# EEGKit/yagi

Hardware: AMD Instinct MI355X
Metric: Msamples/sec, 256-tap firfilt_crcf + 4096-pt FFT stream (higher is better)
Workload: dtype f32

## Files before the change

yagi_amd/csrc/capi.hip:

```cpp
#include <cmath>
#include <cstdlib>
#include <complex>
#include <memory>

#include <algorithm>
#include <atomic>

#include "kernels.hpp"
#include "objstate.hpp"

namespace yagi {

int design_kaiser(size_t n, float fc, float as_, float mu, std::vector<float> &h);
int window_value(int type, size_t i, size_t wlen, float arg, float *out);
int design_notch(size_t m, float f0, float as_, std::vector<float> &h);

static int require_device() {
    static int ok = -1;
    if (ok < 0) {
        int n = 0;
        hipError_t e = hipGetDeviceCount(&n);
        ok = (e == hipSuccess && n > 0) ? 1 : 0;
    }
    if (!ok) return fail(YAGI_ERR_DEVICE, "no HIP device available: libyagi_hip has no CPU fallback");
    return YAGI_OK;
}

template <class V> static V one_of();
template <> float one_of<float>() { return 1.0f; }
template <> cf32 one_of<cf32>() { return cf32{1.0f, 0.0f}; }
static cf32 to_c(float v, cf32 *) { return cf32{v, 0.0f}; }
static float to_c(float v, float *) { return v; }

struct StreamPipe {
    bool on = false;
    static constexpr int kLanes = 2;
    hipStream_t lane[kLanes] = {};
    hipEvent_t in = nullptr, done[kLanes] = {};
    bool busy[kLanes] = {};
    unsigned calls = 0;
    const void *prev_tail = nullptr;
    int init() {
        if (lane[0]) return YAGI_OK;
        for (auto &s : lane) YG_HIP(hipStreamCreateWithFlags(&s, hipStreamNonBlocking));
        YG_HIP(hipEventCreateWithFlags(&in, hipEventDisableTiming));
        for (auto &e : done) YG_HIP(hipEventCreateWithFlags(&e, hipEventDisableTiming));
        return YAGI_OK;
    }
    ~StreamPipe() {
        for (auto &s : lane)
            if (s) { (void)hipStreamSynchronize(s); (void)hipStreamDestroy(s); }
        if (in) (void)hipEventDestroy(in);
        for (auto &e : done) if (e) (void)hipEventDestroy(e);
    }
};

template <class T>
struct DevWindow {
    int len = 0;
    static constexpr int kBufs = 3;
    PingPong<kBufs> ring;
    static constexpr size_t kSlack = 4096;
    std::vector<T> hbuf;
    size_t hend = 0;
    Mirror mirror;
    uint64_t npush = 0;
    StreamPipe pipe;

    int join(hipStream_t st) {
        for (int i = 0; i < StreamPipe::kLanes; ++i) {
            if (pipe.busy[i]) YG_HIP(hipStreamWaitEvent(st, pipe.done[i], 0));
            pipe.busy[i] = false;
        }
        if (pipe.prev_tail) {
            YG_TRY(launch_update_window<T>(dev(), static_cast<const T *>(pipe.prev_tail), (size_t)len, len, next(), st));
            flip();
            pipe.prev_tail = nullptr;
        }
        return YAGI_OK;
    }
    int begin_piped(hipStream_t st, hipStream_t *lane, const T **win) {
        const int i = (int)(pipe.calls % (unsigned)StreamPipe::kLanes);
        YG_HIP(hipEventRecord(pipe.in, st));
        YG_HIP(hipStreamWaitEvent(pipe.lane[i], pipe.in, 0));
        *lane = pipe.lane[i];
        *win = pipe.prev_tail ? static_cast<const T *>(pipe.prev_tail) : dev();
        return YAGI_OK;
    }
    int finish_piped(const T *x, size_t n) {
        const int i = (int)(pipe.calls % (unsigned)StreamPipe::kLanes);
        YG_HIP(hipEventRecord(pipe.done[i], pipe.lane[i]));
        pipe.busy[i] = true;
        ++pipe.calls;
        pipe.prev_tail = x + (n - (size_t)len);
        mirror.dev_written();
        return YAGI_OK;
    }
    bool can_pipe(size_t n) const { return pipe.on && mirror.dev_current() && n >= (size_t)len; }

    int init(int n, hipStream_t st) {
        len = n;
        YG_TRY(ring.alloc((size_t)n * sizeof(T)));
        hbuf.assign((size_t)n + kSlack, T{});
        npush = 0;
        return reset(st);
    }
    int reset(hipStream_t st) {
        YG_TRY(join(st));
        YG_HIP(hipMemsetAsync(ring.cur(), 0, (size_t)len * sizeof(T), st));
        std::fill(hbuf.begin(), hbuf.begin() + len, T{});
        hend = (size_t)len;
        mirror.in_sync();
        return YAGI_OK;
    }
    const T *dev() const { return ring.template cur<T>(); }
    T *next() { return ring.template next<T>(); }
    void flip() { ring.flip(); mirror.dev_written(); }
    int advance(const T *x_dev, size_t n, hipStream_t st) {
        if (n == 0) return YAGI_OK;
        YG_TRY(launch_update_window<T>(dev(), x_dev, n, len, next(), st));
        flip();
        return YAGI_OK;
    }
    const T *host() const { return hbuf.data() + (hend - (size_t)len); }
    void push(T v) {
        if (hend == hbuf.size()) {
            std::memmove(hbuf.data(), hbuf.data() + (hend - (size_t)len + 1), ((size_t)len - 1) * sizeof(T));
            hend = (size_t)len - 1;
        }
        hbuf[hend++] = v;
        ++npush;
        mirror.host_written();
    }
    int ensure_dev(hipStream_t st) {
        YG_TRY(join(st));
        return mirror.need_dev([&] { return upload(ring.cur(), host(), (size_t)len * sizeof(T), st); });
    }
    int ensure_host(hipStream_t st) {
        YG_TRY(join(st));
        return mirror.need_host([&] {
            hend = (size_t)len;
            return download(hbuf.data(), ring.cur(), (size_t)len * sizeof(T), st);
        });
    }
    int clone_from(const DevWindow &o, hipStream_t st) {
        YG_TRY(init(o.len, st));
        YG_HIP(hipMemcpyAsync(ring.cur(), o.ring.cur(), (size_t)len * sizeof(T), hipMemcpyDeviceToDevice, st));
        YG_HIP(hipStreamSynchronize(st));
        npush = o.npush;
        mirror.dev_written();
        return YAGI_OK;
    }
};

template <class T, class C> T host_fir_ring_dot(const T *w, size_t L, size_t head, const C *h, C scale);
template <class T, class C> T host_fir_window_dot(const T *w, size_t L, const C *h, C scale);

template <class K>
struct FirFilt {
    using T = typename K::T;
    using C = typename K::C;
    hipStream_t st = nullptr;
    int L = 0, Lp = 0;
    std::vector<C> h;
    C scale = one_of<C>();
    DevBuf taps;
    DevBuf taps_pad;
    DevBuf apack;
    int Lm = 0;
    DevBuf hfreq, twf, twb;
    DevBuf gfft, gfft_s;
    DevBuf hfreq_s;
    bool hfreq_s_valid = false;
    float hfreq_s_scale = 0.f;
    bool conv_ready = false;
    DevWindow<T> w;
    Staging ws;
    int kernel_choice = 0;
    int prepare_conv();

    int load_taps(const C *hh, size_t n) {
        if (n == 0) return fail(YAGI_ERR_CONFIG, "filter length must be greater than zero");
        if (n > (size_t)1 << 24) return fail(YAGI_ERR_CONFIG, "filter too long");
        h.assign(hh, hh + n);
        L = (int)n;
        YG_TRY(fill(taps, h.data(), n * sizeof(C), st));
        conv_ready = false;
        hfreq_s_valid = false;
        if (K::id == 1) {
            Lp = (L + 31) / 32 * 32;
            std::vector<float> hp((size_t)Lp, 0.0f);
            std::memcpy(hp.data(), h.data(), n * sizeof(float));
            YG_TRY(fill(taps_pad, hp.data(), (size_t)Lp * sizeof(float), st));
            Lm = mfma_lp_for(L);
            if (Lm) {
                std::vector<float> ap(toeplitz_pack_floats(Lm));
                pack_toeplitz_taps(reinterpret_cast<const float *>(h.data()), L, Lm, ap.data());
                YG_TRY(fill(apack, ap.data(), ap.size() * sizeof(float), st));
            }
        }
        return YAGI_OK;
    }
    int init(const C *hh, size_t n) {
        YG_TRY(require_device());
        YG_TRY(load_taps(hh, n));
        return w.init(L, st);
    }
    int block_dev(const T *x, size_t n, T *y);
    T host_execute() const {
        const size_t Ls = (size_t)L, head = (Ls - (size_t)(w.npush % Ls)) % Ls;
        return host_fir_ring_dot<T, C>(w.host(), Ls, head, h.data(), scale);
    }
};

template <class K>
int FirFilt<K>::block_dev(const T *x, size_t n, T *y) {
    if (n == 0) return w.ensure_dev(st);
    const bool piped = w.can_pipe(n) && (kernel_choice != 4 || conv_ready);
    hipStream_t s = st;
    const T *win = nullptr;
    if (piped) YG_TRY(w.begin_piped(st, &s, &win));
    else { YG_TRY(w.ensure_dev(st)); win = w.dev(); }
    T *wnext = piped ? nullptr : w.next();
    w.npush += n;
    const bool conv = kernel_choice == 4 && L <= 2049;
    if (conv) {
        YG_TRY(prepare_conv());
        if constexpr (K::id == 0)
            YG_TRY(launch_fir_rrrf_fftconv(win, x, 0, n, hfreq.as<cf32>(), scale, L, twf.as<cf32>(), twb.as<cf32>(), y, n, s, wnext));
        else
            YG_TRY(launch_fir_cccf_fftconv(win, x, 0, n, hfreq.as<cf32>(), scale, L, twf.as<cf32>(), twb.as<cf32>(), y, n, s, wnext));
    } else {
        YG_TRY((launch_fir_block<K>(win, x, taps.template as<C>(), L, 1, scale, y, n, s, 0, wnext)));
    }
    if (piped) return w.finish_piped(x, n);
    w.flip();
    return YAGI_OK;
}
template <>
int FirFilt<CRCF>::block_dev(const cf32 *x, size_t n, cf32 *y) {
    if (n == 0) return w.ensure_dev(st);
    const bool conv = kernel_choice == 4 && L <= 2049;
    const bool mfma = Lm && (kernel_choice == 3 || (kernel_choice == 0 && n >= ((size_t)1 << 16)));
// ... 1790 lines not shown
        if (q->use_conv) {                                                                          \
            YG_TRY(q->fir.w.ensure_dev(q->st));                                                          \
            YG_TRY(o->fir.w.clone_from(q->fir.w, q->st));                                           \
        } else {                                                                                    \
            YG_HIP(hipMemcpyAsync(o->w.cur(), q->w.cur(), (size_t)q->n * sizeof(cf32),              \
                                  hipMemcpyDeviceToDevice, q->st));                                 \
        YG_HIP(hipStreamSynchronize(q->st));                                                    \
        }                                                                                           \
        *out = o.release();                                                                         \
        return YAGI_OK;                                                                             \
    } catch (...) { return ::yagi::api_exception(); }                                               \
    int yagi_hip_fftfilt_##K##_set_stream(yagi_hip_fftfilt_##K q, yagi_stream_t s) try {            \
        CHECK_Q(q);                                                                                 \
        if (q->st == to_stream(s)) return YAGI_OK;                                                  \
        YG_HIP(hipStreamSynchronize(q->st));                                                        \
        q->st = to_stream(s);                                                                       \
        return YAGI_OK;                                                                             \
    } catch (...) { return ::yagi::api_exception(); }                                               \
    int yagi_hip_fftfilt_##K##_reset(yagi_hip_fftfilt_##K q) try {                                  \
        CHECK_Q(q);                                                                                 \
        return q->reset();                                                                          \
    } catch (...) { return ::yagi::api_exception(); }                                               \
    int yagi_hip_fftfilt_##K##_set_scale(yagi_hip_fftfilt_##K q, C scale) try {                     \
        CHECK_Q(q);                                                                                 \
        q->scale = div_scalar(scale, 2.0f * (float)q->n);                                           \
        return YAGI_OK;                                                                             \
    } catch (...) { return ::yagi::api_exception(); }                                               \
    int yagi_hip_fftfilt_##K##_get_scale(yagi_hip_fftfilt_##K q, C *scale) try {                    \
        CHECK_Q(q);                                                                                 \
        CHECK_PTR(scale);                                                                           \
        *scale = mul_scalar(q->scale, 2.0f * (float)q->n);                                          \
        return YAGI_OK;                                                                             \
    } catch (...) { return ::yagi::api_exception(); }                                               \
    int yagi_hip_fftfilt_##K##_get_length(yagi_hip_fftfilt_##K q, size_t *h_len) try {              \
        CHECK_Q(q);                                                                                 \
        CHECK_PTR(h_len);                                                                           \
        *h_len = q->h.size();                                                                       \
        return YAGI_OK;                                                                             \
    } catch (...) { return ::yagi::api_exception(); }                                               \
    int yagi_hip_fftfilt_##K##_execute(yagi_hip_fftfilt_##K q, const T *x, size_t nx, T *y,         \
                                       size_t ny) try {                                             \
        CHECK_Q(q);                                                                                 \
        if (nx != (size_t)q->n || ny != (size_t)q->n)                                               \
            return fail(YAGI_ERR_CONFIG, "input and output lengths must match filter block size");  \
        CHECK_PTR(x);                                                                               \
        CHECK_PTR(y);                                                                               \
        return q->blocks_host(x, 1, y);                                                             \
    } catch (...) { return ::yagi::api_exception(); }                                               \
    int yagi_hip_fftfilt_##K##_execute_blocks(yagi_hip_fftfilt_##K q, const T *x, size_t nblocks,   \
                                              T *y) try {                                           \
        CHECK_Q(q);                                                                                 \
        if (nblocks == 0) return YAGI_OK;                                                           \
        CHECK_PTR(x);                                                                               \
        CHECK_PTR(y);                                                                               \
        return q->blocks_host(x, nblocks, y);                                                       \
    } catch (...) { return ::yagi::api_exception(); }                                               \
    int yagi_hip_fftfilt_##K##_execute_blocks_dev(yagi_hip_fftfilt_##K q, const T *x,               \
                                                  size_t nblocks, T *y) try {                       \
        CHECK_Q(q);                                                                                 \
        if (nblocks == 0) return YAGI_OK;                                                           \
        CHECK_PTR(x);                                                                               \
        CHECK_PTR(y);                                                                               \
        CHECK_NOALIAS(x, nblocks * (size_t)q->n, y, nblocks * (size_t)q->n);                        \
        return q->blocks_dev(x, nblocks, y);                                                        \
    } catch (...) { return ::yagi::api_exception(); }                                               \
    }

YAGI_FFTFILT_IMPL(rrrf, RRRF, float, float)
YAGI_FFTFILT_IMPL(crcf, CRCF, yagi_cf32, float)
YAGI_FFTFILT_IMPL(cccf, CCCF, yagi_cf32, yagi_cf32)

struct yagi_hip_firfft_crcf_s : FirFft {};

extern "C" {

int yagi_hip_firfft_crcf_create(const float *h, size_t h_len, size_t nfft, yagi_hip_firfft_crcf *q) try {
    CHECK_PTR(q);
    *q = nullptr;
    if (h_len && !h) return fail(YAGI_ERR_CONFIG, "null pointer argument");
    if (nfft == 0) return fail(YAGI_ERR_CONFIG, "fft length must be greater than zero");
    auto o = std::make_unique<yagi_hip_firfft_crcf_s>();
    YG_TRY(o->fir.init(h, h_len));
    if (o->fir.L > 2049) return fail(YAGI_ERR_CONFIG, "fused stream: filter too long (%zu taps, at most 2049)", h_len);
    o->nfft = nfft;
    if (nfft == 4096) YG_TRY(make_stream_twiddles(o->tw));
    else YG_TRY(fft_plan_init(o->plan, nfft, YAGI_FFT_FORWARD));
    *q = o.release();
    return YAGI_OK;
} catch (...) { return ::yagi::api_exception(); }
int yagi_hip_firfft_crcf_destroy(yagi_hip_firfft_crcf q) try { delete q; return YAGI_OK; } catch (...) { return ::yagi::api_exception(); }
int yagi_hip_firfft_crcf_set_pipeline(yagi_hip_firfft_crcf q, int on) try {
    CHECK_Q(q);
    YG_TRY(q->join());
    if (on) YG_TRY(q->fir.w.pipe.init());
    q->fir.w.pipe.on = on != 0;
    return YAGI_OK;
} catch (...) { return ::yagi::api_exception(); }
int yagi_hip_firfft_crcf_join(yagi_hip_firfft_crcf q) try {
    CHECK_Q(q);
    return q->join();
} catch (...) { return ::yagi::api_exception(); }
int yagi_hip_firfft_crcf_set_stream(yagi_hip_firfft_crcf q, yagi_stream_t s) try {
    CHECK_Q(q);
    if (q->fir.st == to_stream(s)) return YAGI_OK;
    YG_TRY(q->join());
    YG_HIP(hipStreamSynchronize(q->fir.st));
    q->fir.st = to_stream(s);
    return YAGI_OK;
} catch (...) { return ::yagi::api_exception(); }
int yagi_hip_firfft_crcf_set_scale(yagi_hip_firfft_crcf q, float scale) try { CHECK_Q(q); q->fir.scale = scale; return YAGI_OK; } catch (...) { return ::yagi::api_exception(); }
int yagi_hip_firfft_crcf_reset(yagi_hip_firfft_crcf q) try {
    CHECK_Q(q);
    YG_TRY(q->join());
    return q->fir.w.reset(q->fir.st);
} catch (...) { return ::yagi::api_exception(); }
int yagi_hip_firfft_crcf_set_variant(yagi_hip_firfft_crcf q, int variant) try {
    CHECK_Q(q);
    if (variant < 0 || variant > 4) return fail(YAGI_ERR_CONFIG, "unknown variant %d", variant);
    if (q->nfft != 4096 && variant != 0 && variant != 3)
        return fail(YAGI_ERR_CONFIG, "nfft = %zu runs as overlap-save FIR + batched FFT (variant 3) only", q->nfft);
    if (variant == 3 && q->fir.L > 2049) return fail(YAGI_ERR_CONFIG, "fast convolution needs <= 2049 taps");
    if (variant == 4 && q->fir.L > 257) return fail(YAGI_ERR_CONFIG, "frequency-domain variant needs <= 257 taps");
    if (variant == 2 && !q->fir.Lm) return fail(YAGI_ERR_CONFIG, "MFMA variant needs <= 256 taps");
    if (variant == 1 && q->fir.Lp > kSlideMaxTaps) return fail(YAGI_ERR_CONFIG, "sliding variant needs <= %d taps", kSlideMaxTaps);
    YG_TRY(q->join());
    q->variant = variant;
    return YAGI_OK;
} catch (...) { return ::yagi::api_exception(); }
int yagi_hip_firfft_crcf_execute_dev(yagi_hip_firfft_crcf q, const yagi_cf32 *x, size_t nframes, yagi_cf32 *spectra) try {
    CHECK_Q(q);
    if (nframes == 0) return YAGI_OK;
    CHECK_PTR(x);
    CHECK_PTR(spectra);
    CHECK_NOALIAS(x, nframes * q->nfft, spectra, nframes * q->nfft);
    auto &f = q->fir;
    const bool use_freq = q->nfft == 4096 && (q->variant == 4 || (q->variant == 0 && f.L <= 257));
    const bool piped = use_freq && f.w.can_pipe(nframes * q->nfft) && f.conv_ready && f.hfreq_s_valid &&
                       f.hfreq_s_scale == f.scale;
    if (!piped) YG_TRY(f.w.ensure_dev(f.st));
    if (q->nfft != 4096) {
        YG_TRY(f.prepare_conv());
        const size_t n = nframes * q->nfft;
        YG_TRY(q->scratch.ensure(n * sizeof(cf32)));
        cf32 *ys = q->scratch.as<cf32>();
        YG_TRY(launch_fir_crcf_fftconv(f.w.dev(), x, 0, n, f.hfreq.as<cf32>(), f.scale, f.L, f.twf.as<cf32>(),
                                       f.twb.as<cf32>(), ys, n, f.st));
        YG_TRY(launch_fft_batch(q->plan.d, ys, spectra, nframes, f.st));
        return f.w.advance(x, n, f.st);
    }
    if (piped) {
        const size_t n = nframes * q->nfft;
        hipStream_t lane;
        const cf32 *win;
        YG_TRY(f.w.begin_piped(f.st, &lane, &win));
        YG_TRY(launch_firfft_crcf_4096_freq(win, x, f.hfreq_s.as<cf32>(), f.gfft_s.as<cf32>(), f.L, q->tw.as<cf32>(), spectra,
                                            nullptr, nframes, lane));
        return f.w.finish_piped(x, n);
    }
    if (use_freq) {
        YG_TRY(f.prepare_conv());
        if (!f.hfreq_s_valid || f.hfreq_s_scale != f.scale) {
            YG_TRY(f.hfreq_s.ensure(4096 * sizeof(cf32)));
            YG_TRY(launch_scale_cf32(f.hfreq.as<cf32>(), f.scale, f.hfreq_s.as<cf32>(), 4096, f.st));
            YG_TRY(f.gfft_s.ensure(512 * sizeof(cf32)));
            YG_TRY(launch_scale_cf32(f.gfft.as<cf32>(), f.scale, f.gfft_s.as<cf32>(), 512, f.st));
            f.hfreq_s_valid = true;
            f.hfreq_s_scale = f.scale;
        }
        YG_TRY(launch_firfft_crcf_4096_freq(f.w.dev(), x, f.hfreq_s.as<cf32>(), f.gfft_s.as<cf32>(), f.L,
                                            q->tw.as<cf32>(), spectra, f.w.next(), nframes, f.st));
        f.w.flip();
        return YAGI_OK;
    }
    const bool use_conv = q->variant == 3 || (q->variant == 0 && f.L <= 2049);
    if (use_conv) {
        YG_TRY(f.prepare_conv());
        const size_t n = nframes * q->nfft;
        YG_TRY(q->scratch.ensure(n * sizeof(cf32)));
        FftPlanDev d;
        d.n = 4096;
        d.dir = YAGI_FFT_FORWARD;
        d.tw = q->tw.as<cf32>();
        cf32 *ys = q->scratch.as<cf32>();
        YG_TRY(launch_fir_crcf_fftconv(f.w.dev(), x, 0, n, f.hfreq.as<cf32>(), f.scale, f.L, f.twf.as<cf32>(),
                                       f.twb.as<cf32>(), ys, n, f.st));
        YG_TRY(launch_fft_batch(d, ys, spectra, nframes, f.st));
        return f.w.advance(x, n, f.st);
    }
    YG_TRY(launch_firfft_crcf_4096(f.w.dev(), x, f.taps_pad.as<float>(), f.apack.as<float>(), f.L, f.Lp, f.Lm, f.scale,
                                   q->tw.as<cf32>(), spectra, nframes, q->variant, f.st));
    return f.w.advance(x, nframes * q->nfft, f.st);
} catch (...) { return ::yagi::api_exception(); }
int yagi_hip_firfft_crcf_execute(yagi_hip_firfft_crcf q, const yagi_cf32 *x, size_t nframes, yagi_cf32 *spectra) try {
    CHECK_Q(q);
    if (nframes == 0) return YAGI_OK;
    CHECK_PTR(x);
    CHECK_PTR(spectra);
    const size_t n = nframes * q->nfft;
    YG_TRY(q->join());
    return q->ws.run(q->fir.st, x, n, spectra, n, [&](const cf32 *xd, cf32 *yd) {
        YG_TRY(yagi_hip_firfft_crcf_execute_dev(q, xd, nframes, yd));
        return q->join();
    });
} catch (...) { return ::yagi::api_exception(); }

}

struct yagi_hip_firpfbch_crcf_s : PfbCh {};
struct yagi_hip_firpfbch2_crcf_s : PfbCh2 {};

extern "C" {

int yagi_hip_firpfbch_crcf_create(size_t M, size_t p, const float *h, yagi_hip_firpfbch_crcf *q) try {
    CHECK_PTR(q);
    *q = nullptr;
    if (M == 0) return fail(YAGI_ERR_CONFIG, "number of channels must be greater than zero");
    if (p == 0) return fail(YAGI_ERR_CONFIG, "invalid filter size (must be greater than 0)");
    CHECK_PTR(h);
    if (M > 8192 || p > 4096) return fail(YAGI_ERR_CONFIG, "channelizer too large");
    YG_TRY(require_device());
    auto o = std::make_unique<yagi_hip_firpfbch_crcf_s>();
    o->M = (int)M;
    o->p = (int)p;
    YG_TRY(fill(o->h, h, M * p * sizeof(float), nullptr));
    YG_TRY(make_twiddles((int)M, YAGI_FFT_FORWARD, o->tw));
    const size_t hl = (p - 1) * M;
    YG_TRY(o->hist.init((int)(hl ? hl : 1), nullptr));
    YG_TRY(o->syn_hist.init((int)(hl ? hl : 1), nullptr));
    *q = o.release();
    return YAGI_OK;
} catch (...) { return ::yagi::api_exception(); }
int yagi_hip_firpfbch_crcf_create_kaiser(size_t M, size_t m, float as_, yagi_hip_firpfbch_crcf *q) try {
    CHECK_PTR(q);
    *q = nullptr;
    if (M == 0) return fail(YAGI_ERR_CONFIG, "number of channels must be greater than zero");
    if (m == 0) return fail(YAGI_ERR_CONFIG, "invalid filter size (must be greater than 0)");
    std::vector<float> hf;
    YG_TRY(design_kaiser(2 * M * m + 1, 0.5f / (float)M, std::fabs(as_), 0.0f, hf));
    return yagi_hip_firpfbch_crcf_create(M, 2 * m, hf.data(), q);
} catch (...) { return ::yagi::api_exception(); }
int yagi_hip_firpfbch_crcf_destroy(yagi_hip_firpfbch_crcf q) try { delete q; return YAGI_OK; } catch (...) { return ::yagi::api_exception(); }
int yagi_hip_firpfbch_crcf_set_stream(yagi_hip_firpfbch_crcf q, yagi_stream_t s) try {
    CHECK_Q(q);
    if (q->st == to_stream(s)) return YAGI_OK;
    YG_HIP(hipStreamSynchronize(q->st));
    q->st = to_stream(s);
    return YAGI_OK;
} catch (...) { return ::yagi::api_exception(); }
int yagi_hip_firpfbch_crcf_reset(yagi_hip_firpfbch_crcf q) try {
    CHECK_Q(q);
    YG_TRY(q->hist.reset(q->st));
    return q->syn_hist.reset(q->st);
} catch (...) { return ::yagi::api_exception(); }
int yagi_hip_firpfbch_crcf_analyzer_execute_dev(yagi_hip_firpfbch_crcf q, const yagi_cf32 *x, size_t nframes, yagi_cf32 *y) try {
    CHECK_Q(q);
    if (nframes == 0) return YAGI_OK;
    CHECK_PTR(x);
    CHECK_PTR(y);
    CHECK_NOALIAS(x, nframes * (size_t)q->M, y, nframes * (size_t)q->M);
    bool written = false;
    cf32 *next = (q->p > 1 && q->hist.len == (int)((q->p - 1) * q->M)) ? q->hist.next() : nullptr;
    YG_TRY(launch_firpfbch(q->hist.dev(), x, q->h.as<float>(), q->M, q->p, q->tw.as<cf32>(), y, nframes, q->st, next, &written));
    if (written) { q->hist.flip(); return YAGI_OK; }
    if (q->p > 1) return q->hist.advance(x, nframes * (size_t)q->M, q->st);
    return YAGI_OK;
} catch (...) { return ::yagi::api_exception(); }
int yagi_hip_firpfbch_crcf_analyzer_execute(yagi_hip_firpfbch_crcf q, const yagi_cf32 *x, size_t nframes, yagi_cf32 *y) try {
    CHECK_Q(q);
    if (nframes == 0) return YAGI_OK;
    CHECK_PTR(x);
    CHECK_PTR(y);
    const size_t n = nframes * (size_t)q->M;
    return q->ws.run(q->st, x, n, y, n,
                     [&](const cf32 *xd, cf32 *yd) { return yagi_hip_firpfbch_crcf_analyzer_execute_dev(q, xd, nframes, yd); });
} catch (...) { return ::yagi::api_exception(); }

int yagi_hip_firpfbch_crcf_synthesizer_execute_dev(yagi_hip_firpfbch_crcf q, const yagi_cf32 *x, size_t nframes, yagi_cf32 *y) try {
    CHECK_Q(q);
    if (nframes == 0) return YAGI_OK;
    CHECK_PTR(x);
    CHECK_PTR(y);
    CHECK_NOALIAS(x, nframes * (size_t)q->M, y, nframes * (size_t)q->M);
    YG_TRY(launch_firpfbch_syn(q->syn_hist.dev(), x, q->h.as<float>(), q->M, q->p, q->tw.as<cf32>(), y, nframes, q->st));
    if (q->p > 1) return q->syn_hist.advance(x, nframes * (size_t)q->M, q->st);
    return YAGI_OK;
} catch (...) { return ::yagi::api_exception(); }
int yagi_hip_firpfbch_crcf_synthesizer_execute(yagi_hip_firpfbch_crcf q, const yagi_cf32 *x, size_t nframes, yagi_cf32 *y) try {
    CHECK_Q(q);
    if (nframes == 0) return YAGI_OK;
    CHECK_PTR(x);
    CHECK_PTR(y);
    const size_t n = nframes * (size_t)q->M;
    return q->ws.run(q->st, x, n, y, n,
                     [&](const cf32 *xd, cf32 *yd) { return yagi_hip_firpfbch_crcf_synthesizer_execute_dev(q, xd, nframes, yd); });
} catch (...) { return ::yagi::api_exception(); }

int yagi_hip_firpfbch2_crcf_create(size_t M, size_t m, const float *h, yagi_hip_firpfbch2_crcf *q) try {
    CHECK_PTR(q);
    *q = nullptr;
    if (M < 2 || (M & 1)) return fail(YAGI_ERR_CONFIG, "number of channels must be greater than 2 and even");
    if (m < 1) return fail(YAGI_ERR_CONFIG, "filter semi-length must be at least 1");
    CHECK_PTR(h);
    if (M > 8192 || m > 2048) return fail(YAGI_ERR_CONFIG, "channelizer too large");
    YG_TRY(require_device());
    auto o = std::make_unique<yagi_hip_firpfbch2_crcf_s>();
    o->M = (int)M;
    o->m = (int)m;
    const size_t hl = 2 * M * m;
    YG_TRY(fill(o->h, h, hl * sizeof(float), nullptr));
    YG_TRY(make_twiddles((int)M, YAGI_FFT_FORWARD, o->tw));
// ... 3653 lines not shown
```

yagi_amd/csrc/devmath.hpp:

```cpp
#pragma once
#include <hip/hip_runtime.h>

#include "common.hpp"

namespace yagi {

template <class T> __device__ __forceinline__ T zero_of();
template <> __device__ __forceinline__ float zero_of<float>() { return 0.0f; }
template <> __device__ __forceinline__ cf32 zero_of<cf32>() { return cf32{0.0f, 0.0f}; }

__device__ __forceinline__ float add(float a, float b) { return a + b; }
__device__ __forceinline__ cf32 add(cf32 a, cf32 b) { return cf32{a.re + b.re, a.im + b.im}; }

__device__ __forceinline__ float mul(float a, float b) { return a * b; }
__device__ __forceinline__ cf32 mul(cf32 a, float b) { return cf32{a.re * b, a.im * b}; }
__device__ __forceinline__ cf32 mul(float a, cf32 b) { return cf32{a * b.re, a * b.im}; }
__device__ __forceinline__ cf32 mul(cf32 a, cf32 b) {
    return cf32{fmaf(a.re, b.re, -a.im * b.im), fmaf(a.re, b.im, a.im * b.re)};
}

__device__ __forceinline__ float mac(float acc, float a, float b) { return fmaf(a, b, acc); }
__device__ __forceinline__ cf32 mac(cf32 acc, cf32 a, float b) {
    return cf32{fmaf(a.re, b, acc.re), fmaf(a.im, b, acc.im)};
}
__device__ __forceinline__ cf32 mac(cf32 acc, float a, cf32 b) {
    return cf32{fmaf(a, b.re, acc.re), fmaf(a, b.im, acc.im)};
}
__device__ __forceinline__ cf32 mac(cf32 acc, cf32 a, cf32 b) {
    return cf32{fmaf(a.re, b.re, fmaf(-a.im, b.im, acc.re)), fmaf(a.re, b.im, fmaf(a.im, b.re, acc.im))};
}

__device__ __forceinline__ float wave_reduce_sum(float v) {
#pragma unroll
    for (int off = 32; off > 0; off >>= 1) v += __shfl_xor(v, off, 64);
    return v;
}
__device__ __forceinline__ cf32 wave_reduce_sum(cf32 v) {
#pragma unroll
    for (int off = 32; off > 0; off >>= 1) {
        v.re += __shfl_xor(v.re, off, 64);
        v.im += __shfl_xor(v.im, off, 64);
    }
    return v;
}

typedef float v2f __attribute__((ext_vector_type(2)));
__device__ __forceinline__ float2 f2(v2f v) { return make_float2(v.x, v.y); }
__device__ __forceinline__ v2f tov(float2 a) { return v2f{a.x, a.y}; }

__device__ __forceinline__ float2 cadd(float2 a, float2 b) { return f2(tov(a) + tov(b)); }
__device__ __forceinline__ float2 csub(float2 a, float2 b) { return f2(tov(a) - tov(b)); }
__device__ __forceinline__ float2 cmul(float2 a, float2 w) {
    v2f r;
    asm("v_pk_mul_f32 %0, %1, %2 op_sel_hi:[0,1]\n\t"
        "v_pk_fma_f32 %0, %1, %2, %0 op_sel:[1,1,0] op_sel_hi:[1,0,1] neg_lo:[0,1,0]"
        : "=&v"(r) : "v"(tov(a)), "v"(tov(w)));
    return f2(r);
}
__device__ __forceinline__ float2 cmul_conj(float2 a, float2 w) {
    v2f r;
    asm("v_pk_mul_f32 %0, %1, %2 op_sel_hi:[0,1] neg_hi:[0,1]\n\t"
        "v_pk_fma_f32 %0, %1, %2, %0 op_sel:[1,1,0] op_sel_hi:[1,0,1]"
        : "=&v"(r) : "v"(tov(a)), "v"(tov(w)));
    return f2(r);
}
template <int SIGN>
__device__ __forceinline__ float2 cmul_dir(float2 a, float2 w) { return SIGN < 0 ? cmul(a, w) : cmul_conj(a, w); }
__device__ __forceinline__ float2 cmul_k(float2 a, float2 k) {
    v2f r;
    asm("v_pk_mul_f32 %0, %1, %2 op_sel_hi:[0,1]\n\t"
        "v_pk_fma_f32 %0, %1, %2, %0 op_sel:[1,1,0] op_sel_hi:[1,0,1] neg_lo:[0,1,0]"
        : "=&v"(r) : "v"(tov(a)), "s"(tov(k)));
    return f2(r);
}
__device__ __forceinline__ float2 cscale(float2 a, float s) { return f2(tov(a) * s); }
__device__ __forceinline__ float2 mul_mi(float2 a) { return make_float2(a.y, -a.x); }
__device__ __forceinline__ float2 mul_pi(float2 a) { return make_float2(-a.y, a.x); }
template <int SIGN>
__device__ __forceinline__ void addsub_rot(float2 a, float2 b, float2 &p, float2 &m) {
    v2f pp, mm;
    if (SIGN < 0) {
        asm("v_pk_add_f32 %0, %1, %2 op_sel:[0,1] op_sel_hi:[1,0] neg_hi:[0,1]" : "=v"(pp) : "v"(tov(a)), "v"(tov(b)));
        asm("v_pk_add_f32 %0, %1, %2 op_sel:[0,1] op_sel_hi:[1,0] neg_lo:[0,1]" : "=v"(mm) : "v"(tov(a)), "v"(tov(b)));
    } else {
        asm("v_pk_add_f32 %0, %1, %2 op_sel:[0,1] op_sel_hi:[1,0] neg_lo:[0,1]" : "=v"(pp) : "v"(tov(a)), "v"(tov(b)));
        asm("v_pk_add_f32 %0, %1, %2 op_sel:[0,1] op_sel_hi:[1,0] neg_hi:[0,1]" : "=v"(mm) : "v"(tov(a)), "v"(tov(b)));
    }
    p = f2(pp);
    m = f2(mm);
}

template <int NT, int B, bool EXACT, class Load, class Store>
__device__ __forceinline__ void batched_for_b(int total, Load load, Store store) {
    using V = decltype(load(0));
    for (int e0 = threadIdx.x; e0 < total; e0 += B * NT) {
        V r[B];
#pragma unroll
        for (int it = 0; it < B; ++it) {
            const int e = e0 + NT * it;
            r[it] = load(EXACT || e < total ? e : total - 1);
        }
#pragma unroll
        for (int it = 0; it < B; ++it) {
            const int e = e0 + NT * it;
            if (EXACT || e < total) store(e, r[it]);
        }
    }
}
template <int NT, class Load, class Store>
__device__ __forceinline__ void batched_for(int total, Load load, Store store) {
    if (total == 8 * NT) batched_for_b<NT, 8, true>(total, load, store);
    else if (total <= 2 * NT) batched_for_b<NT, 2, false>(total, load, store);
    else if (total <= 4 * NT) batched_for_b<NT, 4, false>(total, load, store);
    else batched_for_b<NT, 8, false>(total, load, store);
}

typedef unsigned v2u_t __attribute__((ext_vector_type(2)));
__device__ __forceinline__ __amdgpu_buffer_rsrc_t make_rsrc(const void *p, unsigned bytes) {
    return __builtin_amdgcn_make_buffer_rsrc(const_cast<void *>(p), 0, bytes, 0x00020000);
}
#ifndef YG_STREAM_LD
#define YG_STREAM_LD 16
#endif
#ifndef YG_STREAM_ST
#define YG_STREAM_ST 2
#endif
constexpr int kStreamLoad = YG_STREAM_LD, kStreamStore = YG_STREAM_ST;
__device__ __forceinline__ float2 buf_ld(__amdgpu_buffer_rsrc_t r, unsigned voff, unsigned soff) {
    const v2u_t q = __builtin_amdgcn_raw_buffer_load_b64(r, voff, soff, kStreamLoad);
    return make_float2(__uint_as_float(q.x), __uint_as_float(q.y));
}
template <class T>
__device__ __forceinline__ T ld_stream(const T *p) {
    static_assert(sizeof(T) == 4 || sizeof(T) == 8, "4- or 8-byte samples");
    if constexpr (kStreamLoad == 16) {
        T v;
        if constexpr (sizeof(T) == 4) {
            const unsigned q = __hip_atomic_load(reinterpret_cast<const unsigned *>(p), __ATOMIC_RELAXED, __HIP_MEMORY_SCOPE_AGENT);
            __builtin_memcpy(&v, &q, 4);
        } else {
            const unsigned long long q = __hip_atomic_load(reinterpret_cast<const unsigned long long *>(p), __ATOMIC_RELAXED,
                                                           __HIP_MEMORY_SCOPE_AGENT);
            __builtin_memcpy(&v, &q, 8);
        }
        return v;
    } else {
        return *p;
    }
}
template <class T>
__device__ __forceinline__ void st_stream(T *p, T v) {
    static_assert(sizeof(T) == 4 || sizeof(T) == 8 || sizeof(T) == 16, "4-, 8- or 16-byte samples");
    if constexpr (kStreamStore == 2) {
        typedef float vec_t __attribute__((ext_vector_type(sizeof(T) / 4)));
        vec_t q;
        __builtin_memcpy(&q, &v, sizeof(T));
        __builtin_nontemporal_store(q, reinterpret_cast<vec_t *>(p));
    } else {
        *p = v;
    }
}
template <int AUX>
__device__ __forceinline__ float2 buf_ld_aux(__amdgpu_buffer_rsrc_t r, unsigned voff, unsigned soff) {
    const v2u_t q = __builtin_amdgcn_raw_buffer_load_b64(r, voff, soff, AUX);
    return make_float2(__uint_as_float(q.x), __uint_as_float(q.y));
}
template <int AUX>
__device__ __forceinline__ void buf_st_aux(__amdgpu_buffer_rsrc_t r, unsigned voff, unsigned soff, float2 v) {
    v2u_t q;
    q.x = __float_as_uint(v.x);
    q.y = __float_as_uint(v.y);
    __builtin_amdgcn_raw_buffer_store_b64(q, r, voff, soff, AUX);
}
template <class T>
__device__ __forceinline__ T buf_ld_t(__amdgpu_buffer_rsrc_t r, unsigned voff, unsigned soff) {
    if constexpr (sizeof(T) == 4) {
        const unsigned q = __builtin_amdgcn_raw_buffer_load_b32(r, voff, soff, kStreamLoad);
        T v;
        __builtin_memcpy(&v, &q, 4);
        return v;
    } else {
        static_assert(sizeof(T) == 8, "4- or 8-byte samples");
        const v2u_t q = __builtin_amdgcn_raw_buffer_load_b64(r, voff, soff, kStreamLoad);
        T v;
        __builtin_memcpy(&v, &q, 8);
        return v;
    }
}
__device__ __forceinline__ void buf_st(__amdgpu_buffer_rsrc_t r, unsigned voff, unsigned soff, float2 v) {
    v2u_t q;
    q.x = __float_as_uint(v.x);
    q.y = __float_as_uint(v.y);
    __builtin_amdgcn_raw_buffer_store_b64(q, r, voff, soff, kStreamStore);
}


}
```

yagi_amd/csrc/freq_kernels.hip:

```cpp
#include "fft_core.hpp"
#include "kernels.hpp"

namespace yagi {

constexpr int kFreqMaxTaps = 257;
constexpr unsigned kOffCvs = kFft4096LdsFloat2;
constexpr unsigned kOffT256 = kOffCvs + 256;
constexpr unsigned kFreqLdsFloat2 = kOffT256 + 16 * kTRow;

__device__ __forceinline__ void freq_pass23(float2 (&v)[16], float2 *__restrict__ lds, const float2 *__restrict__ T) {
    const unsigned t = threadIdx.x;
    {
        const unsigned c = t >> 4, bp = t & 15;
#pragma unroll
        for (int a = 0; a < 16; ++a) v[a] = lds[c * kEx1Stride + 16 * a + bp];
        __syncthreads();
        dft16<-1>(v);
#pragma unroll
        for (int cp = 0; cp < 16; ++cp) {
            float2 u = v[dft16_pos(cp)];
            if (cp) u = cmul(u, T[bp * kTRow + cp]);
            lds[bp * kEx2Stride + cp * 16 + c] = u;
        }
    }
    __syncthreads();
    float2 w[16];
#pragma unroll
    for (int bp = 0; bp < 16; ++bp) w[bp] = lds[bp * kEx2Stride + t];
    dft16<-1>(w);
#pragma unroll
    for (int d = 0; d < 16; ++d) v[d] = w[dft16_pos(d)];
    __syncthreads();
}

__device__ __forceinline__ void freq_head256(const float2 *__restrict__ xs, float2 (&v)[16], float2 *__restrict__ lds,
                                             const float2 *__restrict__ T, float2 wbc) {
    const unsigned t = threadIdx.x;
    const unsigned c = t >> 4, bp = t & 15;
    v[0] = xs[bp];
#pragma unroll
    for (int a = 1; a < 16; ++a) v[a] = cmul(xs[16 * a + bp], T[c * kTRow + a]);
    dft16<-1>(v);
#pragma unroll
    for (int cp = 0; cp < 16; ++cp) {
        float2 u = cmul(v[dft16_pos(cp)], wbc);
        if (cp) u = cmul(u, T[bp * kTRow + cp]);
        lds[bp * kEx2Stride + cp * 16 + c] = u;
    }
    __syncthreads();
    float2 w[16];
#pragma unroll
    for (int b = 0; b < 16; ++b) w[b] = lds[b * kEx2Stride + t];
    dft16<-1>(w);
#pragma unroll
    for (int d = 0; d < 16; ++d) v[d] = w[dft16_pos(d)];
}

template <int SIGN>
__device__ __forceinline__ float2 w8(float c, float s) { return make_float2(c, SIGN < 0 ? -s : s); }
template <int SIGN, int NOUT>
__device__ __forceinline__ void dft8_combine(const float2 (&E)[4], float2 (&O)[4], float2 (&X)[8]) {
    const float r2 = 0.70710678118654752f;
    O[1] = cmul_k(O[1], w8<SIGN>(r2, r2));
    O[3] = cmul_k(O[3], w8<SIGN>(-r2, r2));
    X[0] = cadd(E[0], O[0]);
    X[1] = cadd(E[1], O[1]);
    X[3] = cadd(E[3], O[3]);
    if (NOUT > 4) {
        X[4] = csub(E[0], O[0]);
        X[5] = csub(E[1], O[1]);
        X[7] = csub(E[3], O[3]);
        addsub_rot<SIGN>(E[2], O[2], X[2], X[6]);
    } else {
        float2 unused;
        addsub_rot<SIGN>(E[2], O[2], X[2], unused);
    }
}
template <int SIGN, int NIN = 8, int NOUT = 8>
__device__ __forceinline__ void dft8(const float2 (&v)[8], float2 (&X)[8]) {
    float2 E[4], O[4];
    if (NIN == 4) {
        E[0] = cadd(v[0], v[2]); E[2] = csub(v[0], v[2]); addsub_rot<SIGN>(v[0], v[2], E[1], E[3]);
        O[0] = cadd(v[1], v[3]); O[2] = csub(v[1], v[3]); addsub_rot<SIGN>(v[1], v[3], O[1], O[3]);
    } else {
        E[0] = v[0]; E[1] = v[2]; E[2] = v[4]; E[3] = v[6];
        O[0] = v[1]; O[1] = v[3]; O[2] = v[5]; O[3] = v[7];
        dft4<SIGN>(E[0], E[1], E[2], E[3]);
        dft4<SIGN>(O[0], O[1], O[2], O[3]);
    }
    dft8_combine<SIGN, NOUT>(E, O, X);
}
constexpr unsigned kW512S1 = 72, kW512S2 = 68, kW512Ex2 = 8 * kW512S1;
template <int SIGN, int NIN, int NOUT>
__device__ __forceinline__ void wave_fft512(const float2 (&v)[8], float2 (&X)[8], float2 *__restrict__ scr, unsigned l,
                                            float2 w1, float2 w2, float2 w4, float2 u1, float2 u2, float2 u4) {
    float2 z[8], r[8];
    dft8<SIGN, NIN, 8>(v, z);
    {
        const float2 w3 = cmul(w1, w2), w5 = cmul(w4, w1), w6 = cmul(w4, w2), w7 = cmul(w4, w3);
        const float2 w[8] = {w1, w1, w2, w3, w4, w5, w6, w7};
        scr[l] = z[0];
#pragma unroll
        for (int c = 1; c < 8; ++c) scr[c * kW512S1 + l] = cmul_dir<SIGN>(z[c], w[c]);
    }
    __builtin_amdgcn_wave_barrier();
    const unsigned c = l >> 3, bp = l & 7u;
#pragma unroll
    for (int a = 0; a < 8; ++a) r[a] = scr[c * kW512S1 + 8 * a + bp];
    dft8<SIGN, 8, 8>(r, z);
    {
        const float2 u3 = cmul(u1, u2), u5 = cmul(u4, u1), u6 = cmul(u4, u2), u7 = cmul(u4, u3);
        const float2 u[8] = {u1, u1, u2, u3, u4, u5, u6, u7};
        scr[kW512Ex2 + bp * kW512S2 + c] = z[0];
#pragma unroll
        for (int cp = 1; cp < 8; ++cp) scr[kW512Ex2 + bp * kW512S2 + 8 * cp + c] = cmul_dir<SIGN>(z[cp], u[cp]);
    }
    __builtin_amdgcn_wave_barrier();
#pragma unroll
    for (int b = 0; b < 8; ++b) r[b] = scr[kW512Ex2 + b * kW512S2 + l];
    __builtin_amdgcn_wave_barrier();
    dft8<SIGN, 8, NOUT>(r, X);
}

struct CorrOperands {
    float2 dp[4], dq[4];
    float2 w1, w2, w4, u1, u2, u4;
    float2 gc[8];
};
__device__ __forceinline__ void freq_load_corr_fft(CorrOperands &o, const float2 *__restrict__ win,
                                                   const float2 *__restrict__ x, int L, unsigned f,
                                                   const float2 *__restrict__ tw, const float2 *__restrict__ gfft) {
    const unsigned l = threadIdx.x & 63u;
    const int Lc = L - 1;
    const float2 *xf = x + (size_t)f * 4096;
    const float2 *prev = Lc ? (f ? xf - Lc : win + 1) : xf;
    const float2 *own = xf + (4096 - (Lc ? Lc : 1));
#pragma unroll
    for (int a = 0; a < 4; ++a) {
        const unsigned m = 64u * a + l, mi = (int)m < Lc ? m : 0u;
        o.dp[a] = prev[mi];
        o.dq[a] = own[mi];
    }
    o.w1 = tw[8u * l]; o.w2 = tw[16u * l]; o.w4 = tw[32u * l];
    const unsigned bp = l & 7u;
    o.u1 = tw[64u * bp]; o.u2 = tw[128u * bp]; o.u4 = tw[256u * bp];
#pragma unroll
    for (int d = 0; d < 8; ++d) o.gc[d] = gfft[l + 64u * d];
}
__device__ __forceinline__ void freq_correction_fft(const CorrOperands &o, int L, float2 *__restrict__ scr,
                                                    float2 *__restrict__ cvs) {
    const unsigned l = threadIdx.x & 63u;
    const int Lc = L - 1;
    float2 v[8], D[8];
#pragma unroll
    for (int a = 0; a < 4; ++a) v[a] = (int)(64u * a + l) < Lc ? csub(o.dp[a], o.dq[a]) : make_float2(0.f, 0.f);
#pragma unroll
    for (int a = 4; a < 8; ++a) v[a] = make_float2(0.f, 0.f);
    wave_fft512<-1, 4, 8>(v, D, scr, l, o.w1, o.w2, o.w4, o.u1, o.u2, o.u4);
#pragma unroll
    for (int d = 0; d < 8; ++d) v[d] = cmul(D[d], o.gc[d]);
    wave_fft512<1, 8, 4>(v, D, scr, l, o.w1, o.w2, o.w4, o.u1, o.u2, o.u4);
#pragma unroll
    for (int d = 0; d < 4; ++d) cvs[l + 64u * d] = (int)(64u * d + l) < Lc ? D[d] : make_float2(0.f, 0.f);
}

__global__ void __launch_bounds__(256, 4)
firfft_crcf_4096_freq_kernel(const float2 *__restrict__ win, const float2 *__restrict__ x,
                              const float2 *__restrict__ hs, const float2 *__restrict__ gfft, int L,
                              const float2 *__restrict__ tw, float2 *__restrict__ out,
                              float2 *__restrict__ win_next, unsigned nframes) {
    __shared__ __attribute__((aligned(16))) float2 lds[kFreqLdsFloat2];
    float2 *cvs = lds + kOffCvs;
    const float2 *T = lds + kOffT256;
    const float2 *ax = tw + 4096;
    const unsigned t = threadIdx.x, f = blockIdx.x;
    const bool wave0 = __builtin_amdgcn_readfirstlane(t >> 6) == 0;
    const float2 tw_t = ax[1280 + t];
    float2 v[16];
    CorrOperands co;
    if (wave0) freq_load_corr_fft(co, win, x, L, f, tw, gfft);
    __builtin_amdgcn_sched_barrier(0);
    {
        const __amdgpu_buffer_rsrc_t rx = make_rsrc(x + (size_t)f * 4096, 32768u);
#pragma unroll
        for (unsigned a = 0; a < 16; ++a) v[a] = buf_ld(rx, 8u * t, 2048u * a);
    }
    __builtin_amdgcn_sched_barrier(0);
    lds[kOffT256 + (t >> 4) * kTRow + (t & 15u)] = tw_t;
    if (f == nframes - 1 && win_next) {
        const float2 *xf = x + (size_t)f * 4096;
        for (int i = t; i < L; i += 256) win_next[i] = xf[4096 - L + i];
    }
    if (wave0) freq_correction_fft(co, L, lds, cvs);
    __syncthreads();
    dft16<-1>(v);
    {
        float2 w[16];
        twiddle_powers_from(w, ax[t], ax[256 + t], ax[512 + t], ax[768 + t]);
#pragma unroll
        for (int c = 0; c < 16; ++c) {
            float2 z = v[dft16_pos(c)];
            if (c) z = cmul(z, w[c]);
            lds[c * kEx1Stride + t] = z;
        }
    }
    __syncthreads();
    freq_pass23(v, lds, T);
    {
        const __amdgpu_buffer_rsrc_t rh = make_rsrc(hs, 32768u);
        float2 hv[16];
#pragma unroll
        for (unsigned d = 0; d < 16; ++d) hv[d] = buf_ld_aux<0>(rh, 8u * t, 2048u * d);
#pragma unroll
        for (unsigned d = 0; d < 16; ++d) v[d] = cmul(v[d], hv[d]);
    }
    float2 u[16];
    freq_head256(cvs, u, lds, T, ax[1024 + t]);
    const __amdgpu_buffer_rsrc_t ro = make_rsrc(out + (size_t)f * 4096, 32768u);
#pragma unroll
    for (unsigned d = 0; d < 16; ++d)
        buf_st(ro, 8u * t, 2048u * d, make_float2(v[d].x + u[d].x, v[d].y + u[d].y));
}

__global__ void scale_cf32_kernel(const float2 *__restrict__ src, float s, float2 *__restrict__ dst, unsigned n) {
    const unsigned i = blockIdx.x * blockDim.x + threadIdx.x;
    if (i < n) dst[i] = make_float2(src[i].x * s, src[i].y * s);
}
int launch_scale_cf32(const cf32 *src, float s, cf32 *dst, size_t n, hipStream_t st) {
    if (n == 0) return YAGI_OK;
    scale_cf32_kernel<<<(unsigned)((n + 255) / 256), 256, 0, st>>>(reinterpret_cast<const float2 *>(src), s,
                                                                    reinterpret_cast<float2 *>(dst), (unsigned)n);
    YG_LAUNCH_CHECK();
    return YAGI_OK;
}

int launch_firfft_crcf_4096_freq(const cf32 *win, const cf32 *x, const cf32 *hs_scaled, const cf32 *gfft_scaled,
                                 int L, const cf32 *tw_stream, cf32 *spectra, cf32 *win_next, size_t nframes,
                                 hipStream_t st) {
    if (nframes == 0) return YAGI_OK;
    if (L < 1 || L > kFreqMaxTaps)
        return fail(YAGI_ERR_CONFIG, "frequency-domain stream kernel needs 1..%d taps (got %d)", kFreqMaxTaps, L);
    if (nframes > 0x7fffffffull) return fail(YAGI_ERR_CONFIG, "block too large");
    firfft_crcf_4096_freq_kernel<<<(unsigned)nframes, 256, 0, st>>>(
        reinterpret_cast<const float2 *>(win), reinterpret_cast<const float2 *>(x),
        reinterpret_cast<const float2 *>(hs_scaled), reinterpret_cast<const float2 *>(gfft_scaled), L,
        reinterpret_cast<const float2 *>(tw_stream), reinterpret_cast<float2 *>(spectra),
        reinterpret_cast<float2 *>(win_next), (unsigned)nframes);
    YG_LAUNCH_CHECK();
    return YAGI_OK;
}

}
```

Baseline: 303,600.

## Fuse window-tail writes into piped kernel and restructure freq kernel head/tail

```diff
diff --git a/yagi_amd/csrc/capi.hip b/yagi_amd/csrc/capi.hip
--- a/yagi_amd/csrc/capi.hip
+++ b/yagi_amd/csrc/capi.hip
@@ -40,6 +40,7 @@
     bool busy[kLanes] = {};
     unsigned calls = 0;
     const void *prev_tail = nullptr;
+    int made_slot = -1;
     int init() {
         if (lane[0]) return YAGI_OK;
         for (auto &s : lane) YG_HIP(hipStreamCreateWithFlags(&s, hipStreamNonBlocking));
@@ -73,11 +74,23 @@
             pipe.busy[i] = false;
         }
         if (pipe.prev_tail) {
-            YG_TRY(launch_update_window<T>(dev(), static_cast<const T *>(pipe.prev_tail), (size_t)len, len, next(), st));
-            flip();
+            if (pipe.made_slot >= 0) {
+                ring.at = pipe.made_slot;
+                mirror.dev_written();
+            } else {
+                YG_TRY(launch_update_window<T>(dev(), static_cast<const T *>(pipe.prev_tail), (size_t)len, len, next(), st));
+                flip();
+            }
             pipe.prev_tail = nullptr;
+            pipe.made_slot = -1;
         }
         return YAGI_OK;
+    }
+    T *piped_next(int *slot) {
+        static_assert(StreamPipe::kLanes < kBufs, "one ring slot per lane besides the current one");
+        const int i = (int)(pipe.calls % (unsigned)StreamPipe::kLanes);
+        *slot = (ring.at + 1 + i) % kBufs;
+        return static_cast<T *>(ring.buf[*slot].p);
     }
     int begin_piped(hipStream_t st, hipStream_t *lane, const T **win) {
         const int i = (int)(pipe.calls % (unsigned)StreamPipe::kLanes);
@@ -87,8 +100,9 @@
         *win = pipe.prev_tail ? static_cast<const T *>(pipe.prev_tail) : dev();
         return YAGI_OK;
     }
-    int finish_piped(const T *x, size_t n) {
+    int finish_piped(const T *x, size_t n, int made_slot = -1) {
         const int i = (int)(pipe.calls % (unsigned)StreamPipe::kLanes);
+        pipe.made_slot = made_slot;
         YG_HIP(hipEventRecord(pipe.done[i], pipe.lane[i]));
         pipe.busy[i] = true;
         ++pipe.calls;
@@ -2185,10 +2199,12 @@
         const size_t n = nframes * q->nfft;
         hipStream_t lane;
         const cf32 *win;
+        int slot;
         YG_TRY(f.w.begin_piped(f.st, &lane, &win));
+        cf32 *win_next = f.w.piped_next(&slot);
         YG_TRY(launch_firfft_crcf_4096_freq(win, x, f.hfreq_s.as<cf32>(), f.gfft_s.as<cf32>(), f.L, q->tw.as<cf32>(), spectra,
-                                            nullptr, nframes, lane));
-        return f.w.finish_piped(x, n);
+                                            win_next, nframes, lane));
+        return f.w.finish_piped(x, n, slot);
     }
     if (use_freq) {
         YG_TRY(f.prepare_conv());
diff --git a/yagi_amd/csrc/devmath.hpp b/yagi_amd/csrc/devmath.hpp
--- a/yagi_amd/csrc/devmath.hpp
+++ b/yagi_amd/csrc/devmath.hpp
@@ -55,6 +55,13 @@
     asm("v_pk_mul_f32 %0, %1, %2 op_sel_hi:[0,1]\n\t"
         "v_pk_fma_f32 %0, %1, %2, %0 op_sel:[1,1,0] op_sel_hi:[1,0,1] neg_lo:[0,1,0]"
         : "=&v"(r) : "v"(tov(a)), "v"(tov(w)));
+    return f2(r);
+}
+__device__ __forceinline__ float2 cmul_add(float2 a, float2 w, float2 acc) {
+    v2f r;
+    asm("v_pk_fma_f32 %0, %1, %2, %3 op_sel_hi:[0,1,1]\n\t"
+        "v_pk_fma_f32 %0, %1, %2, %0 op_sel:[1,1,0] op_sel_hi:[1,0,1] neg_lo:[0,1,0]"
+        : "=&v"(r) : "v"(tov(a)), "v"(tov(w)), "v"(tov(acc)));
     return f2(r);
 }
 __device__ __forceinline__ float2 cmul_conj(float2 a, float2 w) {
diff --git a/yagi_amd/csrc/freq_kernels.hip b/yagi_amd/csrc/freq_kernels.hip
--- a/yagi_amd/csrc/freq_kernels.hip
+++ b/yagi_amd/csrc/freq_kernels.hip
@@ -30,11 +30,10 @@
     dft16<-1>(w);
 #pragma unroll
     for (int d = 0; d < 16; ++d) v[d] = w[dft16_pos(d)];
-    __syncthreads();
 }
 
 __device__ __forceinline__ void freq_head256(const float2 *__restrict__ xs, float2 (&v)[16], float2 *__restrict__ lds,
-                                             const float2 *__restrict__ T, float2 wbc) {
+                                             const float2 *__restrict__ T, const float2 (&w)[16]) {
     const unsigned t = threadIdx.x;
     const unsigned c = t >> 4, bp = t & 15;
     v[0] = xs[bp];
@@ -42,18 +41,15 @@
     for (int a = 1; a < 16; ++a) v[a] = cmul(xs[16 * a + bp], T[c * kTRow + a]);
     dft16<-1>(v);
 #pragma unroll
-    for (int cp = 0; cp < 16; ++cp) {
-        float2 u = cmul(v[dft16_pos(cp)], wbc);
-        if (cp) u = cmul(u, T[bp * kTRow + cp]);
-        lds[bp * kEx2Stride + cp * 16 + c] = u;
-    }
-    __syncthreads();
-    float2 w[16];
-#pragma unroll
-    for (int b = 0; b < 16; ++b) w[b] = lds[b * kEx2Stride + t];
-    dft16<-1>(w);
-#pragma unroll
-    for (int d = 0; d < 16; ++d) v[d] = w[dft16_pos(d)];
+    for (int cp = 0; cp < 16; ++cp) lds[bp * kEx2Stride + cp * 16 + c] = v[dft16_pos(cp)];
+    __syncthreads();
+    float2 r[16];
+    r[0] = lds[t];
+#pragma unroll
+    for (int b = 1; b < 16; ++b) r[b] = cmul(lds[b * kEx2Stride + t], w[b]);
+    dft16<-1>(r);
+#pragma unroll
+    for (int d = 0; d < 16; ++d) v[d] = r[dft16_pos(d)];
 }
 
 template <int SIGN>
@@ -193,33 +189,27 @@
     }
     if (wave0) freq_correction_fft(co, L, lds, cvs);
     __syncthreads();
+    float2 w[16];
+    twiddle_powers_from(w, ax[t], ax[256 + t], ax[512 + t], ax[768 + t]);
+    float2 u[16];
+    freq_head256(cvs, u, lds, T, w);
+    __syncthreads();
     dft16<-1>(v);
-    {
-        float2 w[16];
-        twiddle_powers_from(w, ax[t], ax[256 + t], ax[512 + t], ax[768 + t]);
-#pragma unroll
-        for (int c = 0; c < 16; ++c) {
-            float2 z = v[dft16_pos(c)];
-            if (c) z = cmul(z, w[c]);
-            lds[c * kEx1Stride + t] = z;
-        }
+#pragma unroll
+    for (int c = 0; c < 16; ++c) {
+        float2 z = v[dft16_pos(c)];
+        if (c) z = cmul(z, w[c]);
+        lds[c * kEx1Stride + t] = z;
     }
     __syncthreads();
     freq_pass23(v, lds, T);
-    {
-        const __amdgpu_buffer_rsrc_t rh = make_rsrc(hs, 32768u);
-        float2 hv[16];
-#pragma unroll
-        for (unsigned d = 0; d < 16; ++d) hv[d] = buf_ld_aux<0>(rh, 8u * t, 2048u * d);
-#pragma unroll
-        for (unsigned d = 0; d < 16; ++d) v[d] = cmul(v[d], hv[d]);
-    }
-    float2 u[16];
-    freq_head256(cvs, u, lds, T, ax[1024 + t]);
+    const __amdgpu_buffer_rsrc_t rh = make_rsrc(hs, 32768u);
     const __amdgpu_buffer_rsrc_t ro = make_rsrc(out + (size_t)f * 4096, 32768u);
-#pragma unroll
-    for (unsigned d = 0; d < 16; ++d)
-        buf_st(ro, 8u * t, 2048u * d, make_float2(v[d].x + u[d].x, v[d].y + u[d].y));
+    float2 hv[16];
+#pragma unroll
+    for (unsigned d = 0; d < 16; ++d) hv[d] = buf_ld_aux<0>(rh, 8u * t, 2048u * d);
+#pragma unroll
+    for (unsigned d = 0; d < 16; ++d) buf_st(ro, 8u * t, 2048u * d, cmul_add(v[d], hv[d], u[d]));
 }
 
 __global__ void scale_cf32_kernel(const float2 *__restrict__ src, float s, float2 *__restrict__ dst, unsigned n) {
```

New measurement: 305,300 (median of 6 runs). About the same (+0.5%).
